# DataIntensive-HPC/abft-sparse-cg

Hardware: AMD Instinct MI355X
Metric: CG iterations/sec + SpMV effective HBM GB/s (% of roofline), 1/2/4/8 MI355X (higher is better)
Workload: dtype f64; 1 GPU; cg-csr -t hip -m none, synthetic laplace5:3162,3162; N=9998244, nnz=49978572, format=csr, mode=none, parallelism=1 GPU

## Files before the change

abft_sparse_cg_amd/capi.py:

```python
import ctypes as C
import os

_HERE = os.path.dirname(os.path.abspath(__file__))
LIB_PATH = os.environ.get("ABFT_HIP_LIB") or os.path.join(_HERE, "libabft_hip.so")
HEADER_PATH = os.path.join(os.path.dirname(_HERE), "include", "abft_hip.h")

OK = 0
MODES = ("none", "constraints", "sed", "sec7", "sec8", "secded")
MODE_ID = {m: i for i, m in enumerate(MODES)}
MODE_ID["sec"] = MODE_ID["sec7"]
FMT_CSR, FMT_COO = 0, 1
FLIP_ANY, FLIP_VALUE, FLIP_INDEX = 0, 1, 2
PART_ALL, PART_INTERIOR, PART_BOUNDARY = 0, 1, 2
K_SPMV, K_DOT, K_CALC_XR, K_CALC_P = 0, 1, 2, 3
EV_VEC_CORRECTED, EV_VEC_DOUBLE = 10, 11
FMT_VECTOR = 2
MAX_RHS = 8

u32p = C.POINTER(C.c_uint32)
f64p = C.POINTER(C.c_double)
i32p = C.POINTER(C.c_int)
vp = C.c_void_p
vpp = C.POINTER(C.c_void_p)

# ... 18 lines not shown
    "abft_hip_shutdown": (C.c_int, [vp]),
    "abft_hip_set_stream": (C.c_int, [vp, vp]),
    "abft_hip_get_stream": (vp, [vp]),
    "abft_hip_synchronize": (C.c_int, [vp]),
    "abft_hip_synchronize_timeout": (C.c_int, [vp, C.c_double]),
    "abft_hip_matrix_create_csr": (C.c_int, [vp, C.c_int, u32p, u32p, f64p, C.c_int, C.c_int, vpp]),
    "abft_hip_matrix_create_coo": (C.c_int, [vp, C.c_int, u32p, u32p, f64p, C.c_int, C.c_int, vpp]),
    "abft_hip_matrix_create_shard": (C.c_int, [vp, C.c_int, C.c_int, u32p, u32p, f64p, C.c_int, C.c_int,
                                               C.c_int, C.c_uint32, vpp]),
    "abft_hip_matrix_create_shard_indexed": (C.c_int, [vp, C.c_int, C.c_int, u32p, u32p, f64p, C.c_int, C.c_int,
                                                       C.c_int, u32p, vpp]),
    "abft_hip_matrix_destroy": (C.c_int, [vp]),
    "abft_hip_matrix_info": (C.c_int, [vp, i32p, i32p]),
    "abft_hip_matrix_compact_stats": (C.c_int, [vp, u32p, u32p, u32p]),
    "abft_hip_matrix_packed_stats": (C.c_int, [vp, u32p, u32p, u32p]),
    "abft_hip_matrix_read_element": (C.c_int, [vp, C.c_uint32, u32p]),
    "abft_hip_matrix_read_csr": (C.c_int, [vp, vp, vp, vp]),
    "abft_hip_matrix_read_coo": (C.c_int, [vp, vp]),
    "abft_hip_inject": (C.c_int, [vp, C.c_uint32, i32p, C.c_int]),
    "abft_hip_inject_rowptr": (C.c_int, [vp, C.c_uint32, C.c_uint32]),
    "abft_hip_vector_create": (C.c_int, [vp, C.c_int, vpp]),
    "abft_hip_vector_view": (C.c_int, [vp, C.c_int, C.c_int, vpp]),
    "abft_hip_vector_destroy": (C.c_int, [vp]),
    "abft_hip_vector_map": (C.c_int, [vp, C.POINTER(f64p)]),
    "abft_hip_vector_unmap": (C.c_int, [vp, f64p]),
    "abft_hip_vector_copy": (C.c_int, [vp, vp]),
    "abft_hip_vector_device_ptr": (vp, [vp]),
    "abft_hip_vector_length": (C.c_int, [vp]),
    "abft_hip_dot": (C.c_int, [vp, vp, vp, f64p]),
    "abft_hip_calc_xr": (C.c_int, [vp, vp, vp, vp, vp, C.c_double, f64p]),
# ... 133 lines not shown
```

abft_sparse_cg_amd/context.py:

```python
import ctypes as C
import math
import sys

import numpy as np

from . import capi
from .capi import FMT_COO, FMT_CSR, MODE_ID, check


class FatalEvent(SystemExit):

    def __init__(self, events):
        super().__init__(1)
        self.events = events


class ResidualCheckFailed(RuntimeError):

    def __init__(self, message, checks):
        super().__init__(message)
        self.checks = checks


class Matrix:
# ... 309 lines not shown
        check(self.L.abft_hip_calc_xr_precond_block(self.h, x.h, r.h, p.h, w.h, dinv.h, k, a.ctypes.data_as(capi.f64p),
                                                    int(active), out.ctypes.data_as(capi.f64p)))
        self._drain_if_pending()
        return out[0::2].copy(), out[1::2].copy()

    def calc_p_precond_block(self, p, r, dinv, k, beta, active):
        b = np.zeros(capi.MAX_RHS)
        b[:k] = beta
        check(self.L.abft_hip_calc_p_precond_block(self.h, p.h, r.h, dinv.h, k, b.ctypes.data_as(capi.f64p),
                                                   int(active)))

    def matrix_info(self, mat):
        lay, n = C.c_int(0), C.c_int(0)
        check(self.L.abft_hip_matrix_info(mat.h, C.byref(lay), C.byref(n)))
        return ("stream", "panels", "sweep", "slice")[lay.value], n.value

    def set_interior(self, mat, row_lo, row_hi):
        check(self.L.abft_hip_matrix_set_interior(mat.h, row_lo, row_hi))

    def inject_bitflip(self, mat, kind, num_flips):
        kind = self.BITFLIP.get(kind, kind)
        rand = self.rng or _libc_rand
        index = rand() % mat.nnz
        if mat.fmt == FMT_CSR:
            start, end = (0, 64) if kind == capi.FLIP_VALUE else (64, 96) if kind == capi.FLIP_INDEX else (0, 96)
        else:
            start, end = (64, 128) if kind == capi.FLIP_VALUE else (0, 64) if kind == capi.FLIP_INDEX else (0, 128)
        bits = []
        for _ in range(num_flips):
            bit = rand() % (end - start) + start
# ... 341 lines not shown
```

abft_sparse_cg_amd/csrc/abft_hip.hip:

```cpp
#include <algorithm>
#include <array>
#include <chrono>
#include <cmath>
#include <cstdarg>
#include <cstdio>
#include <cstdlib>
#include <cstring>
#include <new>
#include <thread>
#include <map>
#include <mutex>
#include <vector>

#include "abft_internal.h"


static thread_local char g_err[512] = "";

static int set_err(int code, const char *fmt, ...) {
  va_list ap;
  va_start(ap, fmt);
  vsnprintf(g_err, sizeof(g_err), fmt, ap);
  va_end(ap);
  return code;
// ... 122 lines not shown
  SweepLayout sweep{};
  int sweep_rpt = 8;
  uint32_t sweep_grid = 0, sweep_width = 0;
  bool use_slice = false;
  SliceLayout slice{};
  uint32_t slice_grid = 0, slice_width = 0;
  std::vector<uint4> blk_host;
  uint32_t t_lo = 0, t_hi = 0;
  CsrCompact compact{};
  std::vector<uint32_t> cbase_host;
  CsrPacked packed{};
  std::vector<uint2> pdesc_host;
  std::vector<uint64_t> pal_host;
  std::map<std::array<uint64_t, ABFT_PAL_ENTRIES>, uint32_t> pal_index;
  size_t pal_cap = 0;
  std::vector<void *> allocs;
};

struct abft_hip_vector {
  abft_hip_ctx *ctx = nullptr;
  double *d = nullptr;
  int n = 0;
  bool owns = true;
  double *host = nullptr;
  abft_hip_vector *root = nullptr;
  bool exposed = false;
  int views = 0;
};

static constexpr uint32_t EVENT_CAP = 1u << 16;
// ... 551 lines not shown
      (m->pal_index.count(pal) || m->pal_host.size() + ABFT_PAL_ENTRIES <= m->pal_cap)) {
    const size_t had = m->pal_host.size();
    d = packed_desc(m, cbase, shift, pal);
    if (m->pal_host.size() > had)
      HIPCHK(hipMemcpyAsync(const_cast<double *>(m->packed.pal) + had, m->pal_host.data() + had,
                            (m->pal_host.size() - had) * 8, hipMemcpyHostToDevice, s));
    HIPCHK(hipMemcpyAsync(const_cast<uint16_t *>(m->packed.code16) + e0, codes.data(), (size_t)n * 2,
                          hipMemcpyHostToDevice, s));
  }
  HIPCHK(hipMemcpyAsync(const_cast<uint2 *>(m->packed.pdesc) + b, &d, sizeof(uint2), hipMemcpyHostToDevice, s));
  HIPCHK(hipStreamSynchronize(s));
  m->pdesc_host[b] = d;
  return ABFT_OK;
}


struct PanelBuild {
  uint32_t ngroups = 0, npanels = 0, width = 0;
  std::vector<uint32_t> seg_base;
  std::vector<uint16_t> seg_ptr;
  std::vector<uint32_t> pos, orig;
};

static bool plan_panels(int mode, const uint32_t *in_idx, const uint32_t *out_idx, int n_out, int n_in, int nnz,
                        PanelBuild &pb, bool constraints_ok = false) {
  const char *env = getenv("ABFT_HIP_LAYOUT");
  const bool force = env && (!strcmp(env, "panels") || !strcmp(env, "sweep"));
  if ((env && !strcmp(env, "stream")) || (mode == ABFT_MODE_CONSTRAINTS && !constraints_ok) || nnz <= 0 || n_out <= 0)
    return false;
  uint32_t width = 1u << 18;
// ... 386 lines not shown
    }
  } else if ((rc = dev_upload(m, &A.cols, columns, (size_t)nnz, padded)) ||
             (rc = dev_upload(m, &A.vals, values, (size_t)nnz, padded))) {
    matrix_free(m);
    return rc;
  }
  if ((rc = dev_upload(m, &d_rowptr, rowptr.data(), rowptr.size(), rowptr.size())) ||
      (rc = dev_upload(m, &d_blk, blk.data(), blk.size(), blk.size()))) {
    matrix_free(m);
    return rc;
  }
  A.rowptr = d_rowptr;
  A.blk = d_blk;
  if (!panels && !sweep && !slice) m->blk_host = blk;
  if (!panels && !sweep && !slice && mode == ABFT_MODE_NONE &&
      ((rc = build_compact_cols(m, columns, blk, padded)) || (rc = build_packed(m, columns, values, blk, padded)))) {
    matrix_free(m);
    return rc;
  }
  hipError_t e = launch_encode_csr(mode, A.cols, A.vals, A.nnz, ctx->stream);
  if (e == hipSuccess) e = hipStreamSynchronize(ctx->stream);
  if (e != hipSuccess) {
    matrix_free(m);
    return set_err(ABFT_ERR_HIP, "CSR upload/encode failed: %s", hipGetErrorString(e));
  }
  *out = m;
  return ABFT_OK;
}

static int create_coo(abft_hip_ctx *ctx, int mode, const uint32_t *columns, const uint32_t *rows,
                      const double *values, int n_out, int n_in, int nnz, uint32_t index_base,
// ... 279 lines not shown
      const uint32_t shift = pdesc[b].y & 31u, pbase = (pdesc[b].y >> 5) * ABFT_PAL_ENTRIES;
      const bool sane = shift >= 12u && shift <= 16u && (size_t)pbase + ABFT_PAL_ENTRIES <= pal.size();
      for (uint32_t i = blk[b].z; i < blk[b].w && i < A.nnz; i++) {
        if (!sane) { bad++; continue; }
        const uint32_t c = pdesc[b].x + (code[i] & ((1u << shift) - 1u));
        bad += c != cols[i] || pal[pbase + (code[i] >> shift)] != vals[i];
      }
    }
  }
  if (packed_tiles) *packed_tiles = np;
  if (tiles) *tiles = stream ? (uint32_t)blk.size() : 0u;
  if (mismatches) *mismatches = bad;
  return ABFT_OK;
}

extern "C" int abft_hip_matrix_destroy(abft_hip_matrix *mat) {
  if (!mat) return ABFT_OK;
  if (int rc = bind(mat->ctx)) return rc;
  HIPCHK(hipStreamSynchronize(mat->ctx->stream));
  matrix_free(mat);
  return ABFT_OK;
}

extern "C" int abft_hip_matrix_read_csr(abft_hip_matrix *mat, uint32_t *cols, uint32_t *rowptr,
                                        double *values) {
  if (!mat || mat->fmt != ABFT_FMT_CSR) return set_err(ABFT_ERR_INVALID, "not a CSR matrix");
  if (int rc = bind(mat->ctx)) return rc;
  hipStream_t s = mat->ctx->stream;
  const CsrDev &A = mat->csr;
  if (rowptr) HIPCHK(hipMemcpyAsync(rowptr, A.rowptr, ((size_t)A.n_out + 1) * 4, hipMemcpyDeviceToHost, s));
// ... 61 lines not shown
  const int width = mat->fmt == ABFT_FMT_CSR ? 96 : 128;
  if (index >= nnz) return set_err(ABFT_ERR_INVALID, "element index %u outside [0,%u)", index, nnz);
  if (nbits < 0 || nbits > 32 || (nbits && !bits)) return set_err(ABFT_ERR_INVALID, "bad bit list");
  for (int k = 0; k < nbits; k++)
    if (bits[k] < 0 || bits[k] >= width) return set_err(ABFT_ERR_INVALID, "bit %d outside [0,%d)", bits[k], width);
  if (!nbits) return ABFT_OK;
  abft_hip_ctx *ctx = mat->ctx;
  HIPCHK(hipMemcpyAsync(ctx->bits_dev, bits, (size_t)nbits * sizeof(int), hipMemcpyHostToDevice, ctx->stream));
  hipError_t e = mat->fmt == ABFT_FMT_CSR
                     ? launch_inject_csr(mat->csr.vals, mat->csr.cols, mat->csr.pos_of_orig, index, ctx->bits_dev, nbits, ctx->stream)
                     : launch_inject_coo(mat->coo.elems, mat->coo.pos_of_orig, index, ctx->bits_dev, nbits, ctx->stream);
  HIPCHK(e);
  HIPCHK(hipStreamSynchronize(ctx->stream));
  bool col_bit = false;
  for (int k = 0; k < nbits; k++) col_bit = col_bit || bits[k] >= 64;
  if (mat->fmt == ABFT_FMT_CSR && mat->compact.cbase && col_bit)
    if (int rc = compact_after_inject(mat, index)) return rc;
  if (mat->fmt == ABFT_FMT_CSR && mat->packed.pdesc) return packed_after_inject(mat, index);
  return ABFT_OK;
}

extern "C" int abft_hip_inject_rowptr(abft_hip_matrix *mat, uint32_t row, uint32_t mask) {
  if (!mat || mat->fmt != ABFT_FMT_CSR) return set_err(ABFT_ERR_INVALID, "not a CSR matrix");
  if (int rc = bind(mat->ctx)) return rc;
  if (row > mat->csr.n_out) return set_err(ABFT_ERR_INVALID, "row pointer %u outside [0,%u]", row, mat->csr.n_out);
  hipStream_t s = mat->ctx->stream;
  uint32_t v = 0;
  uint32_t *p = const_cast<uint32_t *>(mat->csr.rowptr) + row;
  HIPCHK(hipMemcpyAsync(&v, p, sizeof(v), hipMemcpyDeviceToHost, s));
  HIPCHK(hipStreamSynchronize(s));
  v ^= mask;
  HIPCHK(hipMemcpyAsync(p, &v, sizeof(v), hipMemcpyHostToDevice, s));
  HIPCHK(hipStreamSynchronize(s));
  return ABFT_OK;
}


extern "C" int abft_hip_vector_create(abft_hip_ctx *ctx, int N, abft_hip_vector **vec) {
  if (int rc = bind(ctx)) return rc;
  if (!vec || N < 0) return set_err(ABFT_ERR_INVALID, "bad vector arguments");
  abft_hip_vector *v = new (std::nothrow) abft_hip_vector();
  if (!v) return set_err(ABFT_ERR_NOMEM, "vector allocation failed");
  v->ctx = ctx; v->n = N; v->owns = true; v->root = v;
  if (hipMalloc((void **)&v->d, ((size_t)N + 2) * sizeof(double)) != hipSuccess) {
    delete v;
    return set_err(ABFT_ERR_NOMEM, "hipMalloc of %zu bytes failed", ((size_t)N + 2) * sizeof(double));
  }
  *vec = v;
// ... 884 lines not shown
      nparts = mat->panel_grid;
      HIPCHK(launch_spmv_csr_panels(mat->mode, mat->csr, mat->panels, vec->d, result->d, ctx->ring,
                                    do_fuse ? &fuse : nullptr, mat->panel_grid, mat->panel_chunk, ctx->stream));
    } else if (mat->fmt == ABFT_FMT_COO && mat->use_panels) {
      nparts = mat->panel_grid;
      if (mat->coo_pc)
        HIPCHK(launch_spmv_coo_pc(mat->mode, mat->coo, mat->panels, vec->d, result->d, ctx->ring,
                                  do_fuse ? &fuse : nullptr, mat->panel_grid, mat->panel_chunk, ctx->stream));
      else if (mat->coo_lean)
        HIPCHK(launch_spmv_coo_lean(mat->mode, mat->coo, mat->panels, vec->d, result->d, ctx->ring,
                                    do_fuse ? &fuse : nullptr, mat->panel_grid, mat->panel_chunk, ctx->stream));
      else
        HIPCHK(launch_spmv_coo_panels(mat->mode, mat->coo, mat->panels, vec->d, result->d, ctx->ring,
                                      do_fuse ? &fuse : nullptr, mat->panel_grid, mat->panel_chunk, ctx->stream));
    } else if (mat->fmt == ABFT_FMT_CSR)
      HIPCHK(launch_spmv_csr(mat->mode, mat->csr, mat->compact, mat->packed, span, vec->d, result->d, ctx->ring,
                             do_fuse ? &fuse : nullptr, ctx->stream, vecc));
    else
      HIPCHK(launch_spmv_coo(mat->mode, mat->coo, vec->d, result->d, ctx->ring, do_fuse ? &fuse : nullptr, ctx->stream));
    if (mat->fmt == ABFT_FMT_COO) {
      fix = make_fix_args(mat->mode, mat->coo, mat->use_panels ? &mat->panels : nullptr, vec->d, result->d,
                          do_fuse ? &fuse : nullptr);
      if (!do_fuse) HIPCHK(launch_coo_fixup(fix, ctx->stream));
    }
  }
  if (part == ABFT_PART_INTERIOR || !last_range) return ABFT_OK;
  if (do_fuse && hold) {
    hold->held = true;
    hold->fuse = fuse;
    hold->nparts = nparts;
    hold->fix = fix;
// ... 948 lines not shown
```

abft_sparse_cg_amd/csrc/abft_internal.h:

```cpp
#pragma once
#include <hip/hip_runtime.h>
#include <stdint.h>

#include "../../include/abft_hip.h"

struct EventRing {
  abft_event *buf;
  uint32_t *count;
  uint32_t cap;
};

struct CsrDev {
  uint32_t *cols;
  double *vals;
  const uint32_t *rowptr;
  const uint4 *blk;
  uint32_t nblk, n_out, n_in, nnz, index_base;
  const uint32_t *orig_index;
  const uint32_t *pos_of_orig;
  const uint32_t *gidx;
};

#define ABFT_CBASE_WIDE 0xFFFFFFFFu
struct CsrCompact {
  const uint16_t *cols16;
  const uint32_t *cbase;
};

#define ABFT_PAL_ENTRIES 16u
struct CsrPacked {
  const uint16_t *code16;
  const uint2 *pdesc;
  const double *pal;
};

struct CsrPanels {
  const uint32_t *seg_base;
  const uint16_t *seg_ptr;
  uint32_t ngroups, npanels;
  unsigned long long *debug;
  uint32_t *pace;
  uint32_t lag;
  uint32_t width;
  uint32_t xpf;
};
struct SweepLayout {
  const uint32_t *wbase;
  const uint8_t *counts;
// ... 184 lines not shown
                             EventRing ev, const FuseOut *fuse, uint32_t grid, uint32_t c0, uint32_t c1, hipStream_t s);
int spmv_sweep_blocks_per_cu(int mode, int rpt);
hipError_t launch_spmv_slice(int mode, const CsrDev &A, const SliceLayout &L, const double *x, double *y, EventRing ev,
                             const FuseOut *fuse, uint32_t grid, uint32_t c0, uint32_t c1, hipStream_t s);
int spmv_slice_blocks_per_cu(int mode, uint32_t rows_log2);

hipError_t launch_spmv_csr_panels(int mode, const CsrDev &A, const CsrPanels &P, const double *x, double *y,
                                  EventRing ev, const FuseOut *fuse, uint32_t grid, uint32_t chunk,
                                  hipStream_t s);
int spmv_csr_panels_blocks_per_cu(int mode, bool fuse);
hipError_t launch_spmv_coo_panels(int mode, const CooDev &A, const CsrPanels &P, const double *x, double *y,
                                  EventRing ev, const FuseOut *fuse, uint32_t grid, uint32_t chunk,
                                  hipStream_t s);
struct FixArgs;
hipError_t launch_fuse_finalize(const FuseOut &f, uint32_t nblk, const ReduceOut &big, const FixArgs *fix, hipStream_t s);
hipError_t launch_spmv_csr(int mode, const CsrDev &A, const CsrCompact &cc, const CsrPacked &cp, const TileSpan &span,
                           const double *x, double *y, EventRing ev, const FuseOut *fuse, hipStream_t s,
                           bool vecc = false);
hipError_t launch_spmv_coo(int mode, const CooDev &A, const double *x, double *y, EventRing ev,
                           const FuseOut *fuse, hipStream_t s);
struct FixLayout {
  int kind;
  CsrPanels P;
};
struct FixArgs {
  CooDev A;
  FixLayout F;
  const double *x;
  double *y;
  double *partial0;
  uint32_t x_off;
  int ecc;
  int on;
// ... 131 lines not shown
```

abft_sparse_cg_amd/csrc/kernels.hip:

```cpp
#include <type_traits>

#include "abft_internal.h"
#include "ecc_device.h"

typedef double f64x2 __attribute__((ext_vector_type(2)));
typedef uint32_t u32x2 __attribute__((ext_vector_type(2)));
typedef uint32_t u32x4 __attribute__((ext_vector_type(4)));

#if ABFT_CFG_NT
#define STREAM_LOAD(p) __builtin_nontemporal_load(p)
#else
#define STREAM_LOAD(p) (*(p))
#endif

#ifndef ABFT_CFG_GATHER
#define ABFT_CFG_GATHER 0
#endif
__device__ __forceinline__ double gather_load(const double *p) {
#if ABFT_CFG_GATHER == 1
  return __builtin_nontemporal_load(p);
#elif ABFT_CFG_GATHER == 2
  return __hip_atomic_load(p, __ATOMIC_RELAXED, __HIP_MEMORY_SCOPE_AGENT);
#else
  return *p;
// ... 604 lines not shown
                   a3 = s_prod[min(k + 3u, last)];
      acc += a0;
      if (i + 1u < re) acc += a1;
      if (i + 2u < re) acc += a2;
      if (i + 3u < re) acc += a3;
    }
    return true;
  }
  for (uint32_t i = rs; i < re; i++) {
    if (!csr_check_element(A, ev, base, i, re, row_end, s_col, row)) return false;
    acc += s_prod[i - base];
  }
  return true;
}

template <int MODE, int EPT, bool FUSE, bool VECC = false>
__global__ __launch_bounds__(ABFT_BLOCK) void spmv_csr_kernel(CsrDev A, const double *__restrict__ x,
                                                              double *__restrict__ y, EventRing ev,
                                                              FuseOut fuse, TileSpan span, CsrCompact cc,
                                                              CsrPacked cp) {
  constexpr uint32_t TILE = ABFT_BLOCK * EPT;
  __shared__ __attribute__((aligned(16))) double s_prod[TILE];
  __shared__ __attribute__((aligned(16))) uint32_t s_col[MODE == MODE_CONSTRAINTS ? TILE : 2];
  const uint32_t b = xcd_tile(blockIdx.x, span.count);
  const uint32_t t = span.first + b + (b >= span.cut ? span.skip : 0u);
  const uint4 desc = A.blk[t];
  const uint32_t cb = (MODE == MODE_NONE && cc.cbase) ? cc.cbase[t] : ABFT_CBASE_WIDE;
  const uint2 pd = (MODE == MODE_NONE && cp.pdesc) ? cp.pdesc[t] : make_uint2(0u, 0u);
  const bool uniform = ABFT_CFG_UNIFORM_ROWS && MODE != MODE_CONSTRAINTS && (desc.y >> 31) != 0u;
  const uint32_t row0 = desc.x, row1 = desc.y & 0x7fffffffu, e0 = desc.z, e1 = desc.w;
  const uint32_t base = e0 & ~1u;
  double dsum = 0.0;

  if (e1 >= e0 && e1 - base <= TILE) {
    const uint32_t r = row0 + threadIdx.x;
    uint32_t rs = 0, re = 0;
    double xr = 0.0;
    if (r < row1) {
      if (uniform) {
        const uint32_t len = (e1 - e0) / (row1 - row0);
        rs = e0 + len * threadIdx.x; re = rs + len;
      } else {
        rs = A.rowptr[r]; re = A.rowptr[r + 1];
      }
      if (FUSE) xr = x[fuse.x_off + r];
    }
    if (MODE == MODE_NONE && pd.y != 0u)
      csr_stage_packed<EPT, VECC>(A, cp, pd, x, ev, base, e0, e1, s_prod);
    else if (MODE == MODE_NONE)
// ... 46 lines not shown
        if (threadIdx.x == 0 && ok) ok = csr_row_sum<MODE>(A, ev, b, lo, hi, re, s_prod, s_col, acc, row);
        lo = hi;
      }
      if (threadIdx.x == 0 && ok) {
        if (VECC) {
          const uint64_t yw = vecc_encode(acc);
          y[row] = vecc_double(yw);
          if (FUSE) dsum += vecc_decode_cold_ok(x + fuse.x_off + row, fuse.x_off + row, 0u, ev) * vecc_value(yw);
        } else {
          y[row] = acc;
          if (FUSE) dsum += x[fuse.x_off + row] * acc;
        }
      }
    }
  }
  if (FUSE) fused_dot_finish(dsum, fuse, t);
}

template <int MODE, int EPT, bool FUSE>
__global__ __launch_bounds__(ABFT_BLOCK) void spmv_csr_panels_kernel(CsrDev A, CsrPanels P,
                                                                     const double *__restrict__ x,
                                                                     double *__restrict__ y, EventRing ev,
                                                                     FuseOut fuse, uint32_t c0, uint32_t c1) {
  constexpr uint32_t TILE = ABFT_BLOCK * EPT;
  constexpr int RPT = ABFT_PANEL_ROWS_PER_THREAD;
  __shared__ __attribute__((aligned(16))) double s_prod[TILE];
  __shared__ __attribute__((aligned(16))) uint32_t s_col[2];
  double dsum = 0.0;
  for (uint32_t g = blockIdx.x; g < P.ngroups; g += gridDim.x) {
    const uint32_t row0 = g * ABFT_PANEL_ROWS;
    double acc[RPT];
// ... 91 lines not shown
    n = 1;
  return n > 8 ? 8 : n;
}

int spmv_csr_panels_blocks_per_cu(int mode, bool fuse) {
  switch (mode) {
    case MODE_NONE: return fuse ? panels_occupancy<MODE_NONE, true>() : panels_occupancy<MODE_NONE, false>();
    case MODE_SED: return fuse ? panels_occupancy<MODE_SED, true>() : panels_occupancy<MODE_SED, false>();
    case MODE_SEC7: return fuse ? panels_occupancy<MODE_SEC7, true>() : panels_occupancy<MODE_SEC7, false>();
    case MODE_SEC8: return fuse ? panels_occupancy<MODE_SEC8, true>() : panels_occupancy<MODE_SEC8, false>();
    default: return fuse ? panels_occupancy<MODE_SECDED, true>() : panels_occupancy<MODE_SECDED, false>();
  }
}

template <int MODE>
static hipError_t launch_spmv_csr_mode(const CsrDev &A, const CsrCompact &cc, const CsrPacked &cp, const TileSpan &span,
                                       const double *x, double *y, EventRing ev, const FuseOut *fuse, hipStream_t s,
                                       bool vecc) {
  if (vecc && fuse)
    hipLaunchKernelGGL((spmv_csr_kernel<MODE, ABFT_CSR_EPT, true, true>), dim3(span.count), dim3(ABFT_BLOCK), 0, s, A,
                       x, y, ev, *fuse, span, cc, cp);
  else if (vecc)
    hipLaunchKernelGGL((spmv_csr_kernel<MODE, ABFT_CSR_EPT, false, true>), dim3(span.count), dim3(ABFT_BLOCK), 0, s, A,
                       x, y, ev, FuseOut{}, span, cc, cp);
  else if (fuse) {
    hipLaunchKernelGGL((spmv_csr_kernel<MODE, ABFT_CSR_EPT, true>), dim3(span.count), dim3(ABFT_BLOCK), 0, s, A,
                       x, y, ev, *fuse, span, cc, cp);
  } else
    hipLaunchKernelGGL((spmv_csr_kernel<MODE, ABFT_CSR_EPT, false>), dim3(span.count), dim3(ABFT_BLOCK), 0, s, A,
                       x, y, ev, FuseOut{}, span, cc, cp);
  return hipGetLastError();
}

hipError_t launch_spmv_csr(int mode, const CsrDev &A, const CsrCompact &cc, const CsrPacked &cp, const TileSpan &span,
                           const double *x, double *y, EventRing ev, const FuseOut *fuse, hipStream_t s, bool vecc) {
  if (span.count == 0) return hipSuccess;
  if ((uint64_t)span.first + span.count + span.skip > A.nblk || span.cut > span.count) return hipErrorInvalidValue;
  if ((cc.cbase || cc.cols16) && (mode != MODE_NONE || !cc.cbase || !cc.cols16)) return hipErrorInvalidValue;
  if ((cp.code16 || cp.pdesc || cp.pal) && (mode != MODE_NONE || !cp.code16 || !cp.pdesc || !cp.pal))
    return hipErrorInvalidValue;
  switch (mode) {
    case MODE_NONE: return launch_spmv_csr_mode<MODE_NONE>(A, cc, cp, span, x, y, ev, fuse, s, vecc);
    case MODE_CONSTRAINTS: return launch_spmv_csr_mode<MODE_CONSTRAINTS>(A, cc, cp, span, x, y, ev, fuse, s, vecc);
    case MODE_SED: return launch_spmv_csr_mode<MODE_SED>(A, cc, cp, span, x, y, ev, fuse, s, vecc);
    case MODE_SEC7: return launch_spmv_csr_mode<MODE_SEC7>(A, cc, cp, span, x, y, ev, fuse, s, vecc);
    case MODE_SEC8: return launch_spmv_csr_mode<MODE_SEC8>(A, cc, cp, span, x, y, ev, fuse, s, vecc);
    case MODE_SECDED: return launch_spmv_csr_mode<MODE_SECDED>(A, cc, cp, span, x, y, ev, fuse, s, vecc);
    default: return hipErrorInvalidValue;
  }
}

#define SPMM_NO_COL 0xffffffffu

template <int MODE, int EPT>
__device__ __forceinline__ void spmm_stage(const CsrDev &A, const EventRing &ev, uint32_t base, uint32_t lo,
                                           uint32_t hi, double *s_val, uint32_t *s_col) {
  constexpr int STEPS = EPT / 2;
  CsrTileRegs<EPT> t;
  csr_issue_loads<EPT>(A, base, hi, t);
  uint32_t col[EPT];
  double val[EPT];
  uint32_t bad = 0u;
// ... 3781 lines not shown
```

include/abft_hip.h:

```cpp
#ifndef ABFT_HIP_H
#define ABFT_HIP_H

#include <stddef.h>
#include <stdint.h>

#ifdef __cplusplus
extern "C" {
#endif

#define ABFT_OK 0
#define ABFT_ERR_INVALID (-1)
#define ABFT_ERR_HIP (-2)
#define ABFT_ERR_NOMEM (-3)
#define ABFT_ERR_RANGE (-4)
#define ABFT_ERR_NODEVICE (-5)

typedef enum {
  ABFT_MODE_NONE = 0,
  ABFT_MODE_CONSTRAINTS = 1,
  ABFT_MODE_SED = 2,
  ABFT_MODE_SEC7 = 3,
  ABFT_MODE_SEC8 = 4,
  ABFT_MODE_SECDED = 5
} abft_mode;
// ... 49 lines not shown
                               abft_hip_matrix **mat);
int abft_hip_matrix_create_shard(abft_hip_ctx *ctx, int format, int mode,
                                 const uint32_t *columns, const uint32_t *rows,
                                 const double *values, int n_out, int n_in, int nnz,
                                 uint32_t index_base, abft_hip_matrix **mat);
int abft_hip_matrix_create_shard_indexed(abft_hip_ctx *ctx, int format, int mode,
                                         const uint32_t *columns, const uint32_t *rows,
                                         const double *values, int n_out, int n_in, int nnz,
                                         const uint32_t *global_index, abft_hip_matrix **mat);
int abft_hip_matrix_destroy(abft_hip_matrix *mat);
int abft_hip_matrix_info(abft_hip_matrix *mat, int *layout, int *launches_per_spmv);
int abft_hip_matrix_compact_stats(abft_hip_matrix *mat, uint32_t *compact_tiles, uint32_t *tiles,
                                  uint32_t *mismatches);
int abft_hip_matrix_packed_stats(abft_hip_matrix *mat, uint32_t *packed_tiles, uint32_t *tiles,
                                 uint32_t *mismatches);

int abft_hip_matrix_read_csr(abft_hip_matrix *mat, uint32_t *cols, uint32_t *rowptr,
                             double *values);
int abft_hip_matrix_read_coo(abft_hip_matrix *mat, void *elements);

int abft_hip_matrix_read_element(abft_hip_matrix *mat, uint32_t index, uint32_t *words);

int abft_hip_inject(abft_hip_matrix *mat, uint32_t index, const int *bits, int nbits);

int abft_hip_inject_rowptr(abft_hip_matrix *mat, uint32_t row, uint32_t mask);


int abft_hip_vector_create(abft_hip_ctx *ctx, int N, abft_hip_vector **vec);
int abft_hip_vector_view(abft_hip_vector *parent, int offset, int N, abft_hip_vector **vec);
int abft_hip_vector_destroy(abft_hip_vector *vec);
// ... 187 lines not shown
```

Baseline: 4639 CG iterations/s.

## Add deduplicated row-template SpMV path for CSR tiles with repeated row patterns

At matrix build time, rows within single-tile CSR blocks are hashed by their (relative column offset, value) pattern into a small shared template pool. Each block gets a descriptor: uniform (one template for every row) or mixed (a per-row byte code). A new kernel branch then computes the SpMV from the template table instead of streaming the column and value arrays. This is meant to remove most matrix HBM traffic for stencil-like matrices, leaving mainly x and y traffic. It adds host build cost, extra device tables, descriptor demotion on fault injection, and a changed fused-dot partial write path.

```diff
diff --git a/abft_sparse_cg_amd/capi.py b/abft_sparse_cg_amd/capi.py
--- a/abft_sparse_cg_amd/capi.py
+++ b/abft_sparse_cg_amd/capi.py
@@ -56,6 +56,8 @@
     "abft_hip_matrix_info": (C.c_int, [vp, i32p, i32p]),
     "abft_hip_matrix_compact_stats": (C.c_int, [vp, u32p, u32p, u32p]),
     "abft_hip_matrix_packed_stats": (C.c_int, [vp, u32p, u32p, u32p]),
+    "abft_hip_matrix_template_stats": (C.c_int, [vp, u32p, u32p, u32p, u32p, u32p]),
+    "abft_hip_matrix_template_tables": (C.c_int, [vp, u32p, u32p, C.POINTER(C.c_uint8)]),
     "abft_hip_matrix_read_element": (C.c_int, [vp, C.c_uint32, u32p]),
     "abft_hip_matrix_read_csr": (C.c_int, [vp, vp, vp, vp]),
     "abft_hip_matrix_read_coo": (C.c_int, [vp, vp]),
diff --git a/abft_sparse_cg_amd/context.py b/abft_sparse_cg_amd/context.py
--- a/abft_sparse_cg_amd/context.py
+++ b/abft_sparse_cg_amd/context.py
@@ -347,6 +347,21 @@
         lay, n = C.c_int(0), C.c_int(0)
         check(self.L.abft_hip_matrix_info(mat.h, C.byref(lay), C.byref(n)))
         return ("stream", "panels", "sweep", "slice")[lay.value], n.value
+
+    def template_stats(self, mat):
+        v = [C.c_uint32() for _ in range(5)]
+        check(self.L.abft_hip_matrix_template_stats(mat.h, *[C.byref(x) for x in v]))
+        return tuple(x.value for x in v)
+
+    def template_tables(self, mat, n_rows):
+        t = C.c_uint32()
+        check(self.L.abft_hip_matrix_packed_stats(mat.h, None, C.byref(t), None))
+        blocks, tdesc = np.zeros((t.value, 2), np.uint32), np.zeros(t.value, np.uint32)
+        rcode = np.zeros(n_rows, np.uint8)
+        check(self.L.abft_hip_matrix_template_tables(mat.h, blocks.ctypes.data_as(capi.u32p),
+                                                     tdesc.ctypes.data_as(capi.u32p),
+                                                     rcode.ctypes.data_as(C.POINTER(C.c_uint8))))
+        return blocks, tdesc, rcode
 
     def set_interior(self, mat, row_lo, row_hi):
         check(self.L.abft_hip_matrix_set_interior(mat.h, row_lo, row_hi))
diff --git a/abft_sparse_cg_amd/csrc/abft_hip.hip b/abft_sparse_cg_amd/csrc/abft_hip.hip
--- a/abft_sparse_cg_amd/csrc/abft_hip.hip
+++ b/abft_sparse_cg_amd/csrc/abft_hip.hip
@@ -160,6 +160,9 @@
   std::vector<uint64_t> pal_host;
   std::map<std::array<uint64_t, ABFT_PAL_ENTRIES>, uint32_t> pal_index;
   size_t pal_cap = 0;
+  CsrTemplates tpl{};
+  std::vector<uint32_t> tdesc_host;
+  uint32_t tpl_pool = 0;
   std::vector<void *> allocs;
 };
 
@@ -741,6 +744,122 @@
   return ABFT_OK;
 }
 
+static bool block_is_one_tile(const uint4 &d) { return d.w >= d.z && d.w - (d.z & ~1u) <= (uint32_t)ABFT_CSR_TILE; }
+
+static int build_templates(abft_hip_matrix *m, const uint32_t *rowptr, const uint32_t *columns, const double *values,
+                           const std::vector<uint4> &blk) {
+  if (const char *e = getenv("ABFT_HIP_TEMPLATES"))
+    if (!strcmp(e, "0")) return ABFT_OK;
+  const CsrDev &A = m->csr;
+  if (A.n_in == 0) return ABFT_OK;
+  typedef std::array<uint64_t, 1 + 2 * ABFT_TPL_MAX> Key;
+  std::map<Key, uint32_t> index;
+  std::vector<Key> pool, fresh;
+  std::vector<uint32_t> tdesc(blk.size(), 0u);
+  std::vector<uint8_t> rcode((size_t)A.n_out, 0);
+  std::vector<uint32_t> code;
+  bool any = false;
+  for (size_t b = 0; b < blk.size(); b++) {
+    const uint32_t r0 = blk[b].x, r1 = blk[b].y & 0x7fffffffu;
+    if (!block_is_one_tile(blk[b])) continue;
+    fresh.clear();
+    code.assign(r1 - r0, 0u);
+    Key key, last;
+    uint32_t last_code = ~0u;
+    bool ok = true;
+    for (uint32_t r = r0; ok && r < r1; r++) {
+      const uint32_t rs = rowptr[r], re = rowptr[r + 1];
+      if (re - rs > ABFT_TPL_MAX) { ok = false; break; }
+      key.fill(0);
+      key[0] = re - rs;
+      for (uint32_t i = rs; i < re; i++) {
+        if (columns[i] >= A.n_in) { ok = false; break; }
+        key[1 + 2 * (i - rs)] = (uint32_t)(columns[i] - r);
+        memcpy(&key[2 + 2 * (i - rs)], values + i, 8);
+      }
+      if (!ok) break;
+      if (last_code != ~0u && key == last) {
+        code[r - r0] = last_code;
+        continue;
+      }
+      uint32_t c;
+      auto it = index.find(key);
+      if (it != index.end()) {
+        c = it->second;
+      } else {
+        auto f = std::find(fresh.begin(), fresh.end(), key);
+        if (f == fresh.end()) {
+          if (pool.size() + fresh.size() >= ABFT_TPL_POOL) { ok = false; break; }
+          fresh.push_back(key);
+          f = fresh.end() - 1;
+        }
+        c = (uint32_t)(pool.size() + (size_t)(f - fresh.begin()));
+      }
+      code[r - r0] = c;
+      last = key;
+      last_code = c;
+    }
+    if (!ok) continue;
+    for (const Key &k : fresh) {
+      index.emplace(k, (uint32_t)pool.size());
+      pool.push_back(k);
+    }
+    bool same = true;
+    for (uint32_t r = r0; r < r1; r++) {
+      rcode[r] = (uint8_t)code[r - r0];
+      same = same && code[r - r0] == code[0];
+    }
+    tdesc[b] = same ? ABFT_TPL_UNIFORM | (uint32_t)pool[code[0]][0] << 4 | code[0] << 8 : ABFT_TPL_MIXED;
+    any = true;
+  }
+  if (!any) return ABFT_OK;
+  std::vector<uint32_t> tcount(pool.size());
+  std::vector<uint4> tent(pool.size() * ABFT_TPL_MAX, make_uint4(0u, 0u, 0u, 0u));
+  for (size_t k = 0; k < pool.size(); k++) {
+    tcount[k] = (uint32_t)pool[k][0];
+    for (uint32_t j = 0; j < tcount[k]; j++) {
+      const uint64_t v = pool[k][2 + 2 * j];
+      tent[k * ABFT_TPL_MAX + j] = make_uint4((uint32_t)pool[k][1 + 2 * j], 0u, (uint32_t)v, (uint32_t)(v >> 32));
+    }
+  }
+  uint32_t *ddesc = nullptr, *dcount = nullptr;
+  uint8_t *dcode = nullptr;
+  uint4 *dent = nullptr;
+  int rc;
+  if ((rc = dev_upload(m, &ddesc, tdesc.data(), tdesc.size(), tdesc.size())) ||
+      (rc = dev_upload(m, &dcode, rcode.data(), rcode.size(), rcode.size())) ||
+      (rc = dev_upload(m, &dcount, tcount.data(), tcount.size(), tcount.size())) ||
+      (rc = dev_upload(m, &dent, tent.data(), tent.size(), tent.size())))
+    return rc;
+  HIPCHK(hipStreamSynchronize(m->ctx->stream));
+  m->tpl.tdesc = ddesc;
+  m->tpl.rcode = dcode;
+  m->tpl.tcount = dcount;
+  m->tpl.tent = dent;
+  m->tpl_pool = (uint32_t)pool.size();
+  m->tdesc_host = std::move(tdesc);
+  return ABFT_OK;
+}
+
+static int template_demote(abft_hip_matrix *m, size_t b) {
+  if (m->tdesc_host[b] == 0u) return ABFT_OK;
+  hipStream_t s = m->ctx->stream;
+  const uint32_t zero = 0u;
+  HIPCHK(hipMemcpyAsync(const_cast<uint32_t *>(m->tpl.tdesc) + b, &zero, sizeof(zero), hipMemcpyHostToDevice, s));
+  HIPCHK(hipStreamSynchronize(s));
+  m->tdesc_host[b] = 0u;
+  return ABFT_OK;
+}
+
+static int template_after_inject(abft_hip_matrix *m, uint32_t pos) {
+  const std::vector<uint4> &blk = m->blk_host;
+  auto it = std::upper_bound(blk.begin(), blk.end(), pos, [](uint32_t p, const uint4 &d) { return p < d.z; });
+  if (it == blk.begin()) return ABFT_OK;
+  const size_t b = (size_t)(it - blk.begin()) - 1;
+  if (pos >= blk[b].w) return ABFT_OK;
+  return template_demote(m, b);
+}
+
 
 struct PanelBuild {
   uint32_t ngroups = 0, npanels = 0, width = 0;
@@ -1157,7 +1276,8 @@
   A.blk = d_blk;
   if (!panels && !sweep && !slice) m->blk_host = blk;
   if (!panels && !sweep && !slice && mode == ABFT_MODE_NONE &&
-      ((rc = build_compact_cols(m, columns, blk, padded)) || (rc = build_packed(m, columns, values, blk, padded)))) {
+      ((rc = build_compact_cols(m, columns, blk, padded)) || (rc = build_packed(m, columns, values, blk, padded)) ||
+       (rc = build_templates(m, rowptr.data(), columns, values, blk)))) {
     matrix_free(m);
     return rc;
   }
@@ -1467,6 +1587,87 @@
   return ABFT_OK;
 }
 
+extern "C" int abft_hip_matrix_template_stats(abft_hip_matrix *mat, uint32_t *templated_tiles, uint32_t *uniform_tiles,
+                                              uint32_t *eligible_tiles, uint32_t *mismatches,
+                                              uint32_t *pool_templates) {
+  if (!mat) return set_err(ABFT_ERR_INVALID, "null matrix");
+  if (int rc = bind(mat->ctx)) return rc;
+  const bool stream = mat->fmt == ABFT_FMT_CSR && !mat->use_panels && !mat->use_sweep && !mat->use_slice;
+  uint32_t nt = 0, nu = 0, ne = 0, bad = 0;
+  const std::vector<uint4> &blk = mat->blk_host;
+  if (stream)
+    for (const uint4 &d : blk) ne += block_is_one_tile(d);
+  if (stream && mat->tpl.tdesc) {
+    const CsrDev &A = mat->csr;
+    hipStream_t s = mat->ctx->stream;
+    const size_t np = mat->tpl_pool;
+    std::vector<uint32_t> tdesc(blk.size()), tcount(np), cols(A.nnz), rowptr((size_t)A.n_out + 1);
+    std::vector<uint8_t> rcode(A.n_out);
+    std::vector<uint4> tent(np * ABFT_TPL_MAX);
+    std::vector<uint64_t> vals(A.nnz);
+    HIPCHK(hipMemcpyAsync(tdesc.data(), mat->tpl.tdesc, blk.size() * 4, hipMemcpyDeviceToHost, s));
+    HIPCHK(hipMemcpyAsync(rowptr.data(), A.rowptr, rowptr.size() * 4, hipMemcpyDeviceToHost, s));
+    if (A.n_out) HIPCHK(hipMemcpyAsync(rcode.data(), mat->tpl.rcode, (size_t)A.n_out, hipMemcpyDeviceToHost, s));
+    if (np) {
+      HIPCHK(hipMemcpyAsync(tcount.data(), mat->tpl.tcount, np * 4, hipMemcpyDeviceToHost, s));
+      HIPCHK(hipMemcpyAsync(tent.data(), mat->tpl.tent, tent.size() * sizeof(uint4), hipMemcpyDeviceToHost, s));
+    }
+    if (A.nnz) {
+      HIPCHK(hipMemcpyAsync(cols.data(), A.cols, (size_t)A.nnz * 4, hipMemcpyDeviceToHost, s));
+      HIPCHK(hipMemcpyAsync(vals.data(), A.vals, (size_t)A.nnz * 8, hipMemcpyDeviceToHost, s));
+    }
+    HIPCHK(hipStreamSynchronize(s));
+    for (size_t b = 0; b < blk.size(); b++) {
+      const uint32_t td = tdesc[b];
+      if (td == 0u) continue;
+      nt++;
+      const bool uni = (td & 15u) == ABFT_TPL_UNIFORM;
+      nu += uni;
+      for (uint32_t r = blk[b].x; r < (blk[b].y & 0x7fffffffu); r++) {
+        const uint32_t k = uni ? td >> 8 : rcode[r], rs = rowptr[r], re = rowptr[r + 1];
+        bool same = k < np && rs <= re && re <= A.nnz && tcount[k] == re - rs && tcount[k] <= ABFT_TPL_MAX &&
+                    (!uni || ((td >> 4) & 15u) == tcount[k]);
+        for (uint32_t j = 0; same && j < re - rs; j++) {
+          const uint4 e = tent[(size_t)k * ABFT_TPL_MAX + j];
+          const uint32_t c = r + e.x;
+          same = c < A.n_in && c == cols[rs + j] && ((uint64_t)e.w << 32 | e.z) == vals[rs + j];
+        }
+        bad += !same;
+      }
+    }
+  }
+  if (templated_tiles) *templated_tiles = nt;
+  if (uniform_tiles) *uniform_tiles = nu;
+  if (eligible_tiles) *eligible_tiles = ne;
+  if (mismatches) *mismatches = bad;
+  if (pool_templates) *pool_templates = stream ? mat->tpl_pool : 0u;
+  return ABFT_OK;
+}
+
+extern "C" int abft_hip_matrix_template_tables(abft_hip_matrix *mat, uint32_t *blocks, uint32_t *tdesc,
+                                               uint8_t *rcode) {
+  if (!mat) return set_err(ABFT_ERR_INVALID, "null matrix");
+  if (int rc = bind(mat->ctx)) return rc;
+  const bool stream = mat->fmt == ABFT_FMT_CSR && !mat->use_panels && !mat->use_sweep && !mat->use_slice;
+  const size_t nb = stream ? mat->blk_host.size() : 0, nr = stream ? mat->csr.n_out : 0;
+  hipStream_t s = mat->ctx->stream;
+  if (blocks)
+    for (size_t b = 0; b < nb; b++) {
+      blocks[2 * b] = mat->blk_host[b].x;
+      blocks[2 * b + 1] = mat->blk_host[b].y & 0x7fffffffu;
+    }
+  if (tdesc && nb) {
+    if (mat->tpl.tdesc) HIPCHK(hipMemcpyAsync(tdesc, mat->tpl.tdesc, nb * 4, hipMemcpyDeviceToHost, s));
+    else memset(tdesc, 0, nb * 4);
+  }
+  if (rcode && nr) {
+    if (mat->tpl.rcode) HIPCHK(hipMemcpyAsync(rcode, mat->tpl.rcode, nr, hipMemcpyDeviceToHost, s));
+    else memset(rcode, 0, nr);
+  }
+  HIPCHK(hipStreamSynchronize(s));
+  return ABFT_OK;
+}
+
 extern "C" int abft_hip_matrix_destroy(abft_hip_matrix *mat) {
   if (!mat) return ABFT_OK;
   if (int rc = bind(mat->ctx)) return rc;
@@ -1558,6 +1759,8 @@
   HIPCHK(hipStreamSynchronize(ctx->stream));
   bool col_bit = false;
   for (int k = 0; k < nbits; k++) col_bit = col_bit || bits[k] >= 64;
+  if (mat->fmt == ABFT_FMT_CSR && mat->tpl.tdesc)
+    if (int rc = template_after_inject(mat, index)) return rc;
   if (mat->fmt == ABFT_FMT_CSR && mat->compact.cbase && col_bit)
     if (int rc = compact_after_inject(mat, index)) return rc;
   if (mat->fmt == ABFT_FMT_CSR && mat->packed.pdesc) return packed_after_inject(mat, index);
@@ -1576,6 +1779,12 @@
   v ^= mask;
   HIPCHK(hipMemcpyAsync(p, &v, sizeof(v), hipMemcpyHostToDevice, s));
   HIPCHK(hipStreamSynchronize(s));
+  if (mat->tpl.tdesc)
+    for (size_t b = 0; b < mat->blk_host.size(); b++) {
+      const uint4 &d = mat->blk_host[b];
+      if (d.x <= row && row <= (d.y & 0x7fffffffu))
+        if (int rc = template_demote(mat, b)) return rc;
+    }
   return ABFT_OK;
 }
 
@@ -2490,7 +2699,7 @@
         HIPCHK(launch_spmv_coo_panels(mat->mode, mat->coo, mat->panels, vec->d, result->d, ctx->ring,
                                       do_fuse ? &fuse : nullptr, mat->panel_grid, mat->panel_chunk, ctx->stream));
     } else if (mat->fmt == ABFT_FMT_CSR)
-      HIPCHK(launch_spmv_csr(mat->mode, mat->csr, mat->compact, mat->packed, span, vec->d, result->d, ctx->ring,
+      HIPCHK(launch_spmv_csr(mat->mode, mat->csr, mat->compact, mat->packed, mat->tpl, span, vec->d, result->d, ctx->ring,
                              do_fuse ? &fuse : nullptr, ctx->stream, vecc));
     else
       HIPCHK(launch_spmv_coo(mat->mode, mat->coo, vec->d, result->d, ctx->ring, do_fuse ? &fuse : nullptr, ctx->stream));
diff --git a/abft_sparse_cg_amd/csrc/abft_internal.h b/abft_sparse_cg_amd/csrc/abft_internal.h
--- a/abft_sparse_cg_amd/csrc/abft_internal.h
+++ b/abft_sparse_cg_amd/csrc/abft_internal.h
@@ -32,6 +32,17 @@
   const uint16_t *code16;
   const uint2 *pdesc;
   const double *pal;
+};
+
+#define ABFT_TPL_MAX 8u
+#define ABFT_TPL_POOL 256u
+#define ABFT_TPL_UNIFORM 1u
+#define ABFT_TPL_MIXED 2u
+struct CsrTemplates {
+  const uint32_t *tdesc;
+  const uint8_t *rcode;
+  const uint32_t *tcount;
+  const uint4 *tent;
 };
 
 struct CsrPanels {
@@ -246,9 +257,9 @@
                                   hipStream_t s);
 struct FixArgs;
 hipError_t launch_fuse_finalize(const FuseOut &f, uint32_t nblk, const ReduceOut &big, const FixArgs *fix, hipStream_t s);
-hipError_t launch_spmv_csr(int mode, const CsrDev &A, const CsrCompact &cc, const CsrPacked &cp, const TileSpan &span,
-                           const double *x, double *y, EventRing ev, const FuseOut *fuse, hipStream_t s,
-                           bool vecc = false);
+hipError_t launch_spmv_csr(int mode, const CsrDev &A, const CsrCompact &cc, const CsrPacked &cp, const CsrTemplates &ct,
+                           const TileSpan &span, const double *x, double *y, EventRing ev, const FuseOut *fuse,
+                           hipStream_t s, bool vecc = false);
 hipError_t launch_spmv_coo(int mode, const CooDev &A, const double *x, double *y, EventRing ev,
                            const FuseOut *fuse, hipStream_t s);
 struct FixLayout {
diff --git a/abft_sparse_cg_amd/csrc/kernels.hip b/abft_sparse_cg_amd/csrc/kernels.hip
--- a/abft_sparse_cg_amd/csrc/kernels.hip
+++ b/abft_sparse_cg_amd/csrc/kernels.hip
@@ -642,25 +642,96 @@
   return true;
 }
 
+template <int N, bool FUSE>
+__device__ __forceinline__ void csr_rows_uniform(const CsrTemplates &ct, uint32_t tno, const double *__restrict__ x,
+                                                 double *__restrict__ y, const FuseOut &fuse, uint32_t row0,
+                                                 uint32_t row1, double &dsum) {
+  uint4 e[N ? N : 1];
+#pragma unroll
+  for (int j = 0; j < N; j++) e[j] = ct.tent[tno * ABFT_TPL_MAX + (uint32_t)j];
+  for (uint32_t row = row0 + threadIdx.x; row < row1; row += ABFT_BLOCK) {
+    double xv[N ? N : 1];
+#pragma unroll
+    for (int j = 0; j < N; j++) xv[j] = gather_load(x + (row + e[j].x));
+    double xr = 0.0;
+    if (FUSE) xr = x[fuse.x_off + row];
+    double acc = 0.0;
+#pragma unroll
+    for (int j = 0; j < N; j++) acc += as_double(e[j].z, e[j].w) * xv[j];
+    y[row] = acc;
+    if (FUSE) dsum += xr * acc;
+  }
+}
+
+template <bool FUSE>
+__device__ __forceinline__ void csr_rows_mixed(const CsrTemplates &ct, const double *__restrict__ x,
+                                               double *__restrict__ y, const FuseOut &fuse, uint32_t row0,
+                                               uint32_t row1, double &dsum) {
+  constexpr int N = (int)ABFT_TPL_MAX;
+  for (uint32_t row = row0 + threadIdx.x; row < row1; row += ABFT_BLOCK) {
+    const uint32_t tno = ct.rcode[row];
+    const uint32_t n = ct.tcount[tno];
+    uint4 e[N];
+#pragma unroll
+    for (int j = 0; j < N; j++) e[j] = ct.tent[tno * ABFT_TPL_MAX + (uint32_t)j];
+    double xv[N];
+#pragma unroll
+    for (int j = 0; j < N; j++) xv[j] = gather_load(x + ((uint32_t)j < n ? row + e[j].x : 0u));
+    double xr = 0.0;
+    if (FUSE) xr = x[fuse.x_off + row];
+    double acc = 0.0;
+#pragma unroll
+    for (int j = 0; j < N; j++) {
+      const double sum = acc + as_double(e[j].z, e[j].w) * xv[j];
+      acc = (uint32_t)j < n ? sum : acc;
+    }
+    y[row] = acc;
+    if (FUSE) dsum += xr * acc;
+  }
+}
+
+template <bool FUSE>
+__device__ __forceinline__ void csr_rows_templated(const CsrTemplates &ct, uint32_t td, const double *__restrict__ x,
+                                                   double *__restrict__ y, const FuseOut &fuse, uint32_t row0,
+                                                   uint32_t row1, double &dsum) {
+  const uint32_t tno = td >> 8;
+  if ((td & 15u) == ABFT_TPL_MIXED) return csr_rows_mixed<FUSE>(ct, x, y, fuse, row0, row1, dsum);
+  switch ((td >> 4) & 15u) {
+    case 0: return csr_rows_uniform<0, FUSE>(ct, tno, x, y, fuse, row0, row1, dsum);
+    case 1: return csr_rows_uniform<1, FUSE>(ct, tno, x, y, fuse, row0, row1, dsum);
+    case 2: return csr_rows_uniform<2, FUSE>(ct, tno, x, y, fuse, row0, row1, dsum);
+    case 3: return csr_rows_uniform<3, FUSE>(ct, tno, x, y, fuse, row0, row1, dsum);
+    case 4: return csr_rows_uniform<4, FUSE>(ct, tno, x, y, fuse, row0, row1, dsum);
+    case 5: return csr_rows_uniform<5, FUSE>(ct, tno, x, y, fuse, row0, row1, dsum);
+    case 6: return csr_rows_uniform<6, FUSE>(ct, tno, x, y, fuse, row0, row1, dsum);
+    case 7: return csr_rows_uniform<7, FUSE>(ct, tno, x, y, fuse, row0, row1, dsum);
+    default: return csr_rows_uniform<8, FUSE>(ct, tno, x, y, fuse, row0, row1, dsum);
+  }
+}
+
 template <int MODE, int EPT, bool FUSE, bool VECC = false>
 __global__ __launch_bounds__(ABFT_BLOCK) void spmv_csr_kernel(CsrDev A, const double *__restrict__ x,
                                                               double *__restrict__ y, EventRing ev,
                                                               FuseOut fuse, TileSpan span, CsrCompact cc,
-                                                              CsrPacked cp) {
+                                                              CsrPacked cp, CsrTemplates ct) {
   constexpr uint32_t TILE = ABFT_BLOCK * EPT;
   __shared__ __attribute__((aligned(16))) double s_prod[TILE];
   __shared__ __attribute__((aligned(16))) uint32_t s_col[MODE == MODE_CONSTRAINTS ? TILE : 2];
+  __shared__ double s_wf[4];
   const uint32_t b = xcd_tile(blockIdx.x, span.count);
   const uint32_t t = span.first + b + (b >= span.cut ? span.skip : 0u);
   const uint4 desc = A.blk[t];
   const uint32_t cb = (MODE == MODE_NONE && cc.cbase) ? cc.cbase[t] : ABFT_CBASE_WIDE;
   const uint2 pd = (MODE == MODE_NONE && cp.pdesc) ? cp.pdesc[t] : make_uint2(0u, 0u);
+  const uint32_t td = (MODE == MODE_NONE && !VECC && ct.tdesc) ? ct.tdesc[t] : 0u;
   const bool uniform = ABFT_CFG_UNIFORM_ROWS && MODE != MODE_CONSTRAINTS && (desc.y >> 31) != 0u;
   const uint32_t row0 = desc.x, row1 = desc.y & 0x7fffffffu, e0 = desc.z, e1 = desc.w;
   const uint32_t base = e0 & ~1u;
   double dsum = 0.0;
 
-  if (e1 >= e0 && e1 - base <= TILE) {
+  if (MODE == MODE_NONE && !VECC && td != 0u) {
+    csr_rows_templated<FUSE>(ct, td, x, y, fuse, row0, row1, dsum);
+  } else if (e1 >= e0 && e1 - base <= TILE) {
     const uint32_t r = row0 + threadIdx.x;
     uint32_t rs = 0, re = 0;
     double xr = 0.0;
@@ -737,7 +808,10 @@
       }
     }
   }
-  if (FUSE) fused_dot_finish(dsum, fuse, t);
+  if (FUSE) {
+    const double bsum = block_sum(dsum, s_wf);
+    if (threadIdx.x == 0) fuse.partials[t] = bsum;
+  }
 }
 
 template <int MODE, int EPT, bool FUSE>
@@ -859,38 +933,43 @@
 }
 
 template <int MODE>
-static hipError_t launch_spmv_csr_mode(const CsrDev &A, const CsrCompact &cc, const CsrPacked &cp, const TileSpan &span,
+static hipError_t launch_spmv_csr_mode(const CsrDev &A, const CsrCompact &cc, const CsrPacked &cp, const CsrTemplates &ct,
+                                       const TileSpan &span,
                                        const double *x, double *y, EventRing ev, const FuseOut *fuse, hipStream_t s,
                                        bool vecc) {
   if (vecc && fuse)
     hipLaunchKernelGGL((spmv_csr_kernel<MODE, ABFT_CSR_EPT, true, true>), dim3(span.count), dim3(ABFT_BLOCK), 0, s, A,
-                       x, y, ev, *fuse, span, cc, cp);
+                       x, y, ev, *fuse, span, cc, cp, ct);
   else if (vecc)
     hipLaunchKernelGGL((spmv_csr_kernel<MODE, ABFT_CSR_EPT, false, true>), dim3(span.count), dim3(ABFT_BLOCK), 0, s, A,
-                       x, y, ev, FuseOut{}, span, cc, cp);
+                       x, y, ev, FuseOut{}, span, cc, cp, ct);
   else if (fuse) {
     hipLaunchKernelGGL((spmv_csr_kernel<MODE, ABFT_CSR_EPT, true>), dim3(span.count), dim3(ABFT_BLOCK), 0, s, A,
-                       x, y, ev, *fuse, span, cc, cp);
+                       x, y, ev, *fuse, span, cc, cp, ct);
   } else
     hipLaunchKernelGGL((spmv_csr_kernel<MODE, ABFT_CSR_EPT, false>), dim3(span.count), dim3(ABFT_BLOCK), 0, s, A,
-                       x, y, ev, FuseOut{}, span, cc, cp);
-  return hipGetLastError();
-}
-
-hipError_t launch_spmv_csr(int mode, const CsrDev &A, const CsrCompact &cc, const CsrPacked &cp, const TileSpan &span,
+                       x, y, ev, FuseOut{}, span, cc, cp, ct);
+  return hipGetLastError();
+}
+
+hipError_t launch_spmv_csr(int mode, const CsrDev &A, const CsrCompact &cc, const CsrPacked &cp, const CsrTemplates &ct,
+                                       const TileSpan &span,
                            const double *x, double *y, EventRing ev, const FuseOut *fuse, hipStream_t s, bool vecc) {
   if (span.count == 0) return hipSuccess;
   if ((uint64_t)span.first + span.count + span.skip > A.nblk || span.cut > span.count) return hipErrorInvalidValue;
   if ((cc.cbase || cc.cols16) && (mode != MODE_NONE || !cc.cbase || !cc.cols16)) return hipErrorInvalidValue;
   if ((cp.code16 || cp.pdesc || cp.pal) && (mode != MODE_NONE || !cp.code16 || !cp.pdesc || !cp.pal))
     return hipErrorInvalidValue;
+  if ((ct.tdesc || ct.rcode || ct.tcount || ct.tent) &&
+      (mode != MODE_NONE || !ct.tdesc || !ct.rcode || !ct.tcount || !ct.tent))
+    return hipErrorInvalidValue;
   switch (mode) {
-    case MODE_NONE: return launch_spmv_csr_mode<MODE_NONE>(A, cc, cp, span, x, y, ev, fuse, s, vecc);
-    case MODE_CONSTRAINTS: return launch_spmv_csr_mode<MODE_CONSTRAINTS>(A, cc, cp, span, x, y, ev, fuse, s, vecc);
-    case MODE_SED: return launch_spmv_csr_mode<MODE_SED>(A, cc, cp, span, x, y, ev, fuse, s, vecc);
-    case MODE_SEC7: return launch_spmv_csr_mode<MODE_SEC7>(A, cc, cp, span, x, y, ev, fuse, s, vecc);
-    case MODE_SEC8: return launch_spmv_csr_mode<MODE_SEC8>(A, cc, cp, span, x, y, ev, fuse, s, vecc);
-    case MODE_SECDED: return launch_spmv_csr_mode<MODE_SECDED>(A, cc, cp, span, x, y, ev, fuse, s, vecc);
+    case MODE_NONE: return launch_spmv_csr_mode<MODE_NONE>(A, cc, cp, ct, span, x, y, ev, fuse, s, vecc);
+    case MODE_CONSTRAINTS: return launch_spmv_csr_mode<MODE_CONSTRAINTS>(A, cc, cp, ct, span, x, y, ev, fuse, s, vecc);
+    case MODE_SED: return launch_spmv_csr_mode<MODE_SED>(A, cc, cp, ct, span, x, y, ev, fuse, s, vecc);
+    case MODE_SEC7: return launch_spmv_csr_mode<MODE_SEC7>(A, cc, cp, ct, span, x, y, ev, fuse, s, vecc);
+    case MODE_SEC8: return launch_spmv_csr_mode<MODE_SEC8>(A, cc, cp, ct, span, x, y, ev, fuse, s, vecc);
+    case MODE_SECDED: return launch_spmv_csr_mode<MODE_SECDED>(A, cc, cp, ct, span, x, y, ev, fuse, s, vecc);
     default: return hipErrorInvalidValue;
   }
 }
diff --git a/include/abft_hip.h b/include/abft_hip.h
--- a/include/abft_hip.h
+++ b/include/abft_hip.h
@@ -87,6 +87,9 @@
                                   uint32_t *mismatches);
 int abft_hip_matrix_packed_stats(abft_hip_matrix *mat, uint32_t *packed_tiles, uint32_t *tiles,
                                  uint32_t *mismatches);
+int abft_hip_matrix_template_stats(abft_hip_matrix *mat, uint32_t *templated_tiles, uint32_t *uniform_tiles,
+                                   uint32_t *eligible_tiles, uint32_t *mismatches, uint32_t *pool_templates);
+int abft_hip_matrix_template_tables(abft_hip_matrix *mat, uint32_t *blocks, uint32_t *tdesc, uint8_t *rcode);
 
 int abft_hip_matrix_read_csr(abft_hip_matrix *mat, uint32_t *cols, uint32_t *rowptr,
                              double *values);
```

Result: faster. 4892 CG iterations/s, median of 6 (+5.4%).
